# tkoz0/linear-program-solver

Measured on AMD Instinct MI355X. Metric: pivots/sec + achieved HBM GB/s on dense float64 tableau, 1/2/4/8 MI355X, higher is better.
Workload: dtype f64

## Files before the change

include/lpgpu_diag.h:

```cpp
#ifndef LPGPU_DIAG_H
#define LPGPU_DIAG_H

#include "lpgpu.h"

#ifdef __cplusplus
extern "C" {
#endif

int lpdiag_geometry(lp_handle *h, long long *out );

int lpdiag_sweep_buffers(const lp_handle *h, int *nbuf);

int lpdiag_sweep_clocks(lp_handle *h, unsigned long long *out , int cap, int *n);

int lpdiag_sweep_block_clocks(lp_handle *h, unsigned long long *out , int cap, int *n);

int lpdiag_set_xcd_shards(lp_handle *h, int on);

int lpdiag_stamps(lp_handle *h, long long *out );
int lpdiag_bstamps(lp_handle *h, long long *out );

#ifdef __cplusplus
}
#endif

#endif
```

linear-program-solver_amd/csrc/engine.h:

```cpp
#pragma once

#include <hip/hip_runtime.h>
#include <stdint.h>

#include "../../include/lpgpu.h"
#include "geometry.h"

namespace lpk {

constexpr int MODE_RUN = 0;
constexpr int MODE_SOLVE = 1;

constexpr int RATIO_FULL = 0;
constexpr int RATIO_LOCAL = 1;
constexpr int RATIO_CHECK = 2;

constexpr int RSRC_RECORDS = 0;
constexpr int RSRC_GIVEN = 1;
constexpr int RSRC_SLOTS = 2;
constexpr int RSRC_BAND = 3;

constexpr int ST_STRADDLE = 3;

constexpr int PICK_RATIO = 0;
constexpr int PICK_CHECK = 1;
constexpr int PICK_EXPLICIT = 2;
// ... 85 lines not shown
    int gmaj;
    lp_tol tol;
    long long *stamps;
    unsigned long long *gran;
    unsigned spin_max;
    unsigned xwait_ms;
    int fault;
    int hier;
    int rank;
    int xtarget;
    int share;
    int fault_xcc;
    unsigned long long *xbuf;
    unsigned long long *const *peer;
    double *Tout;
    unsigned *dflips;
    unsigned flipseq;
    unsigned long long *sweep_clk;
    unsigned sweep_lseq;
};
constexpr int SWEEP_CLK_RING = 1024;
constexpr int SWEEP_BLK_MAX = 8192;

constexpr int NRANK_MAX = 64;
constexpr long long XS_SUM_PAR = (NRANK_MAX + 1) * 8;
constexpr long long XS_XREP = 2 * XS_SUM_PAR;
constexpr long long XS_PROW = 8 * XS_XREP;
constexpr long long XS_PROW_BLOCK = 2 * 4 * 64;
constexpr long long XS_PROW_RANK = 256 * XS_PROW_BLOCK;
__host__ __device__ inline long long xs_granules(int nranks)
{
    return XS_PROW + 2LL * nranks * XS_PROW_RANK + 256 * 8;
}

hipError_t launch_reset(hipStream_t s, const Args &A, int mode, int rule, int chain, long long cap,
                        long long r, long long c);
hipError_t launch_load_eager(hipStream_t s, const Args &A);
hipError_t launch_enter(hipStream_t s, const Args &A);
hipError_t launch_ratio(hipStream_t s, const Args &A, int t, int grp, int mode, int from_erec,
                        long long check_local_row);
hipError_t launch_pick(hipStream_t s, const Args &A, int t, int mode);
hipError_t launch_gather(hipStream_t s, const Args &A, int t);
hipError_t launch_prow(hipStream_t s, const Args &A, int t, int grp, int rsrc, int peek);
hipError_t launch_sweep(hipStream_t s, const Args &A, int grp, int nd_max, int cnt = -1, hipEvent_t e0 = nullptr,
                        hipEvent_t e1 = nullptr, bool *flipped = nullptr);

constexpr int GRAN_REGIONS = 4;
constexpr long long GRAN_SHARD = (long long)GRAN_REGIONS * GROUP_MAXBLOCKS * 8;
constexpr long long XS_READER_STRIDE = 1032;
constexpr long long GRAN_TOTAL = (XS_SHARDS + 2) * GRAN_SHARD;
GroupGeom group_geom(long long rc, long long ld, long long n, int bmax, int xr, int nshard, int share,
                     bool xs_ok = true);
const void *sel_kernel(int ipl, int nb, bool xr, bool xs);
int persistent_occupancy(const Variant &v);
hipError_t launch_sel(hipStream_t s, const Args &A, const GroupGeom &geo, int grp, int count, int from_erec,
                      unsigned seq, int xr, int first, int fmode, int frule, long long fcap, hipEvent_t e0,
                      hipEvent_t e1);
hipError_t launch_group(hipStream_t s, const Args &A, const GroupGeom &geo, int grp, int count,
                        int from_erec, unsigned seq, int bmax, int xr, const Args *As, int nshard,
                        int first, int fmode, int frule, long long fcap, hipEvent_t e0 = nullptr,
                        hipEvent_t e1 = nullptr);
hipError_t launch_persistent(const void *fn, dim3 grid, void **args, size_t lds, hipStream_t s, hipEvent_t e0,
                             hipEvent_t e1);
hipError_t launch_peer_ping(hipStream_t s, const Args &A, unsigned tag, unsigned flags, int *ok_dev);
hipError_t launch_group_min(hipStream_t s, double *const *ptrs, int n);

struct ColStat {
    double gmin;
// ... 24 lines not shown
```

linear-program-solver_amd/csrc/geometry.h:

```cpp
#pragma once

#include <algorithm>
#include <cstdint>
#include <functional>

#ifdef __HIP__
#define LPK_HD __host__ __device__
#else
#define LPK_HD
#endif

namespace lpk {

constexpr int BMAX = 64;

constexpr int GROUP_MAXBLOCKS = 256;
constexpr int XS_SHARDS = 8;
constexpr int GROUP_MINBLOCKS = 64;
constexpr int GROUP_THREADS = 64;
constexpr int GROUP_MAXRPL = 4;
constexpr long long GROUP_LDS_MAX = 96 * 1024;
LPK_HD inline long long group_lds(long long rc, long long ld, long long g, int count)
{
    const long long rpb = (rc + g - 1) / g, cpb = (ld + g - 1) / g;
// ... 112 lines not shown
            }
        }
        const long long tail = spread ? ((S.rows + nrun * nsg - 1) / (nrun * nsg) + 7) / 8 * 8 : 0;
        return SweepPlan{K, nsg, nrun, run, runb, na, tail, nfull * 64 * WL, ncol, nrun * nsg};
    }
    constexpr int RW = 4;
    const long long ns = (S.ld + 127) / 128;
    const long long slots = (long long)E.cus * bpc;
    const bool tailed = ns >= 2 && (E.tail_mode == 2 || (E.tail_mode == 1 && S.rows * (ns - 1) >= 2048 * slots));
    const long long nsg = tailed ? ns - 1 : ns;
    long long nrun = slots / nsg;
    if (nrun < 1) nrun = 1;
    long long run = (S.rows + nrun - 1) / nrun;
    run = (run + RW - 1) / RW * RW;
    nrun = (S.rows + run - 1) / run;
    const long long tail = tailed ? ((S.rows + nrun * nsg - 1) / (nrun * nsg) + RW - 1) / RW * RW : 0;
    return SweepPlan{K, nsg, nrun, run, run, (int)nrun, tail, 0, 0, nrun * nsg};
}

inline SweepPlan plan_sweep(const SweepShape &S, const SweepEnv &E)
{
    return plan_sweep_grid(S, choose_sweep_kernel(S), E);
}

struct Variant {
    bool sel;
    int nr, ipl;
    int rpl;
    bool xr, xs, hk;
    size_t lds;
};
constexpr int OCC_MISSING = -(1 << 30);
using Occupancy = std::function<int(const Variant &)>;

inline GroupGeom plan_sel(long long rc, long long n, int bmax, int xcd_cus, bool xr, bool xs_ok, int share,
                          const Occupancy &occ)
{
    GroupGeom G;
    if (rc < 1 || n < 1 || bmax < 1 || bmax > BMAX) return G;
    int xs = 0;
    long long rps = rc;
    if ((rc + 63) / 64 > 64) {
        if (!xs_ok || bmax <= 32) return G;
        xs = XS_SHARDS;
        rps = (rc + XS_SHARDS - 1) / XS_SHARDS;
    }
// ... 109 lines not shown
```

linear-program-solver_amd/csrc/kernels.hip:

```cpp
#include "engine.h"
#include "device.h"
#include "knobs.h"

#include <hip/hip_ext.h>

#include <array>
#include <map>
#include <mutex>

namespace lpk {



__global__ void k_reset(Args A, int mode, int rule, int chain, long long cap, long long r,
                        long long c)
{
    Ctl *ctl = A.ctl;
    ctl->status = LP_PIVOTED;
    ctl->mode = mode;
    ctl->rule = rule;
    ctl->chain = chain;
    ctl->cap = cap;
    ctl->r = r;
    ctl->c = c;
// ... 1563 lines not shown
    while (h) {
        int ra32, rb32;
        const int sa = next_pivot_row(h, mysr, ra32);
        const bool two = h != 0;
        const int sb = two ? next_pivot_row(h, mysr, rb32) : sa;
        if (!two) rb32 = ra32;
        const long long ra_ = ra32, rb_ = rb32;
        double ma[NK], mb[NK];
#pragma unroll
        for (int k = 0; k < NK; ++k) {
            ma[k] = M[mq(ra_, 16 * k + (lane & 15))];
            mb[k] = M[mq(rb_, 16 * k + (lane & 15))];
        }
        double ya = P[(long long)sa * ld + col], yb = P[(long long)sb * ld + col];
        fix_chain_dpp<NB>(ya, ma, p, sa);
        if (ok) Tout[ra_ * ld + col] = ya;
        if (two) {
            fix_chain_dpp<NB>(yb, mb, p, sb);
            if (ok) Tout[rb_ * ld + col] = yb;
        }
    }
}

constexpr int SWEEP_LA = 0;
constexpr int SWEEP_LA_T = 0;
constexpr int SWEEP_LA_OOP = 2;
constexpr bool SWEEP_RGQ = true;
template <int W, int NB, int D, int SA>
__global__ void __launch_bounds__(64 * W)
k_sweep_rl(const double *T, double *Tout, const double *__restrict__ P, const double *__restrict__ M,
           const long long *__restrict__ dR, const Ctl *__restrict__ ctl, long long ld, long long rows, int grp,
           int nstrips, long long run, long long tail, long long tcol, long long tend, int nexp,
           unsigned *dflips, unsigned flipseq, unsigned long long *clk, unsigned lseq, long long runb, int na)
{
    constexpr int RW = 8;
    constexpr int NC = NB / 2;
    constexpr int XS = W * RW * 64;
    constexpr int LAT = (SA & 2) ? SWEEP_LA_OOP : SWEEP_LA_T;
    constexpr int SWEEP_QP = 16;
    constexpr int QP = (D * (XS + 2 * 4 * BMAX + SWEEP_QP) * 8 + 8 * NB <= 80 * 1024 || W > 4) ? SWEEP_QP : 0;
    constexpr int MS = 2 * 4 * BMAX + QP;
    static_assert(NB % 2 == 0 && NB <= BMAX && D >= 2 && W >= 4, "k_sweep_rl");
    __shared__ __attribute__((aligned(16))) double xs[D][XS];
    __shared__ __attribute__((aligned(16))) double ms[D][MS];
    __shared__ long long sr[NB];
    constexpr int LDS_BASE = D * (XS + MS) * 8 + NB * 8;
    constexpr int NF = (W <= 4 && LDS_BASE + 64 * (NB * 8 + 4) <= 80 * 1024) ? 64 : 16;
    __shared__ __attribute__((aligned(16))) double fixm[NF][NB];
    __shared__ int fmeta[NF];
    const int nd = (int)ctl->ndef[grp];
    if (nd == 0 || ctl->bar_timeout) return;
    const int lane = threadIdx.x & 63;
    const int wave = __builtin_amdgcn_readfirstlane(threadIdx.x >> 6);
    if (dflips && blockIdx.x == 0 && threadIdx.x == 0) *dflips = flipseq;
    const unsigned long long clk_c0 = __builtin_amdgcn_s_memtime(), clk_r0 = __builtin_amdgcn_s_memrealtime();
    if (threadIdx.x < NB) sr[threadIdx.x] = (int)threadIdx.x < nd ? dR[threadIdx.x] : -2;
    auto srow = [&](int s) -> long long { return sr[s]; };
    const int strip = (int)(blockIdx.x % (unsigned)nstrips);
    const long long ri = (long long)(blockIdx.x / (unsigned)nstrips);
    const long long r0 = ri < na ? ri * run : (long long)na * run + (ri - na) * runb;
    const long long r1 = min(rows, r0 + (ri < na ? run : runb));
    const long long colw = (long long)strip * 64 * W + 64 * wave;
    const long long col = min(colw + (lane & ~1), ld - 2) + (lane & 1);
    const bool cok = colw + lane < ld;
    const long long t0 = (long long)blockIdx.x * tail, t1 = tail > 0 ? min(rows, t0 + tail) : 0;
    const long long tc = min(tcol + lane, ld - 1);
    const bool tok = tcol + lane < ld;
    if (nd != nexp) {
        __syncthreads();
        auto one = [&](long long row, long long c, bool ok) {
            double x = T[row * ld + c];
            for (int s = 0; s < nd; ++s) {
                if (srow(s) == row) x = P[(long long)s * ld + c];
                else x = fma(-M[mq(row, s)], P[(long long)s * ld + c], x);
            }
            if (ok) Tout[row * ld + c] = x;
        };
        for (long long row = r0; row < r1; ++row) one(row, col, cok);
        for (long long row = t0 + wave; row < t1; row += W) one(row, tc, tok);
        return;
    }
    double p[NB];
#pragma unroll
    for (int s = 0; s < NB; ++s) p[s] = P[(long long)s * ld + col];
// ... 120 lines not shown
    for (int f = 0; f < nf; ++f) {
        int meta;
        double mk[NK];
        meta = __builtin_amdgcn_readfirstlane(fmeta[f]);
#pragma unroll
        for (int k = 0; k < NK; ++k) mk[k] = fixm[f][16 * k + (lane & 15)];
        const int s0 = meta & 255;
        double y = pick_p<0, NB, NB>(p, s0);
        fix_chain_dpp<NB>(y, mk, p, s0);
        if (cok) Tout[(r0 + (meta >> 8)) * ld + col] = y;
    }
    if (ovf) fix_rows<NB>(P, M, Tout, ld, col, cok, p, mysr, r0, r1, 0, 0, ovf);
    if (clk && threadIdx.x == 0) {
        const unsigned long long c1 = __builtin_amdgcn_s_memtime(), rt1 = __builtin_amdgcn_s_memrealtime();
        if (blockIdx.x == 0) {
            unsigned long long *e = clk + (lseq % SWEEP_CLK_RING) * 4;
            e[1] = c1 - clk_c0;
            e[2] = rt1 - clk_r0;
            e[3] = clk_r0;
            e[0] = lseq;
        }
        if (blockIdx.x < SWEEP_BLK_MAX) {
            unsigned long long *e = clk + SWEEP_CLK_RING * 4 + blockIdx.x * 4;
            e[0] = lseq;
            e[1] = clk_r0;
            e[2] = rt1;
            e[3] = c1 - clk_c0;
        }
    }
    if (t0 >= t1) return;
    if (tend - tcol <= 4 && t1 - t0 <= 64LL * W) {
        if (64 * wave < t1 - t0) {
            const long long rw = t0 + 64 * wave + lane;
            const bool rok = rw < t1;
            const long long rr = rok ? rw : t1 - 1;
            const int rri = (int)rr;
            double m[NB];
#pragma unroll
            for (int s = 0; s < NB; ++s) m[s] = M[mq(rr, s)];
            const bool tpiv = __ballot(mysr >= t0 && mysr < t1) != 0;
            for (long long c = tcol; c < tend; ++c) {
                double x = T[rr * ld + c];
                const double pv = lane < NB ? P[(long long)lane * ld + c] : 0.0;
                if (tpiv) {
#pragma unroll
                    for (int s = 0; s < NB; ++s) {
                        const double ps = readlane_f64(pv, s);
                        x = rri == __builtin_amdgcn_readlane((int)(unsigned)mysr, s) ? ps : fma(-m[s], ps, x);
                    }
                } else {
// ... 266 lines not shown
    auto it = cache.find(fn);
    if (it != cache.end()) return it->second;
    int n = 0;
    if (hipOccupancyMaxActiveBlocksPerMultiprocessor(&n, fn, threads, 0) != hipSuccess || n < 1) {
        (void)hipGetLastError();
        n = 1;
    }
    cache[fn] = n;
    return n;
}

static const void *sweep_kernel(const SweepKernel &K)
{
    constexpr int SA = 16, WV = 10;
    if (K.rl)
        return K.W == 8 ? (K.oop ? (const void *)&k_sweep_rl<8, 64, 4, SA | 2> : (const void *)&k_sweep_rl<8, 64, 4, SA>)
                        : (K.oop ? (const void *)&k_sweep_rl<4, 64, 2, SA | 2> : (const void *)&k_sweep_rl<4, 64, 2, SA>);
    return K.nb == 16 ? (const void *)&k_sweep_dp2<WV, 16, SA>
         : K.nb == 32 ? (const void *)&k_sweep_dp2<WV, 32, SA>
         : K.nb == 48 ? (const void *)&k_sweep_dp2<WV, 48, SA>
                      : (const void *)&k_sweep_dp2<WV, 64, SA>;
}

hipError_t launch_sweep(hipStream_t s, const Args &A, int grp, int nd_max, int cnt, hipEvent_t e0, hipEvent_t e1,
                        bool *flipped)
{
    if (flipped) *flipped = false;
    const ProcessKnobs &knobs = process_knobs();
    const SweepShape shape{A.rows, A.n, A.ld, nd_max, cnt, A.share, A.Tout && A.Tout != A.T};
    const SweepKernel K = choose_sweep_kernel(shape);
    const void *fn = sweep_kernel(K);
    const SweepEnv env{sweep_grid_cus(), sweep_blocks_per_cu(fn, 64 * K.W), knobs.sweep_tail, knobs.sweep_split};
    SweepPlan pl = plan_sweep_grid(shape, K, env);
    if (K.nexp < K.nb) {
        hipError_t e = hipMemsetAsync(A.P + (long long)K.nexp * A.ld, 0, (size_t)(K.nb - K.nexp) * A.ld * 8, s);
        if (e == hipSuccess)
            e = hipMemset2DAsync(A.MQ + K.nexp * 4, 4 * BMAX * 8, 0, (size_t)(K.nb - K.nexp) * 4 * 8,
                                 (size_t)((A.rows + 3) / 4), s);
        if (e != hipSuccess) return e;
    }
    const dim3 grid((unsigned)pl.grid);
    const double *T = A.T, *Pp = A.P, *Mp = A.MQ;
    double *To = K.oop ? A.Tout : A.T;
    const long long *dRp = A.dR;
    const Ctl *ctlp = A.ctl;
    long long ld = A.ld, rows = A.rows;
    int grpv = grp, nsv = (int)pl.nsg, nexp = K.nexp;
    unsigned *dfl = K.oop ? A.dflips : nullptr;
    unsigned fseq = A.flipseq;
    unsigned long long *clk = A.sweep_clk;
    unsigned lseq = A.sweep_lseq;
    void *args[] = {&T, &To, &Pp, &Mp, &dRp, &ctlp, &ld, &rows, &grpv, &nsv, &pl.run, &pl.tail, &pl.tcol, &pl.tend,
                    &nexp, &dfl, &fseq, &clk, &lseq, &pl.runb, &pl.na};
    const hipError_t err = hipExtLaunchKernel(fn, grid, dim3(64 * K.W), args, 0, s, e0, e1, 0);
    if (err == hipSuccess && flipped) *flipped = K.oop;
    return err != hipSuccess ? err : hipGetLastError();
}

static const void *group_kernel(int nr, int ipl, int rpl, bool xr, bool hk = false)
{
#define X(NRV, IPLV, RPLV)                                                                     \
    if (nr == NRV && ipl == IPLV && rpl == RPLV)                                               \
        return xr ? reinterpret_cast<const void *>(&k_group<NRV, IPLV, RPLV, true>)            \
             : hk ? reinterpret_cast<const void *>(&k_group<NRV, IPLV, RPLV, false, true>)     \
                  : reinterpret_cast<const void *>(&k_group<NRV, IPLV, RPLV, false>);
    GROUP_VARIANTS(X)
#undef X
    return nullptr;
}

static int persistent_per_cu(const void *fn, size_t lds)
{
    int n = 0;
    if (hipOccupancyMaxActiveBlocksPerMultiprocessor(&n, fn, GROUP_THREADS, lds) != hipSuccess) {
        (void)hipGetLastError();
        return 0;
// ... 86 lines not shown
```

linear-program-solver_amd/csrc/knobs.h:

```cpp
#pragma once

#include <cstdio>
#include <cstdlib>
#include <cstring>

#ifndef LPK_TEAM_WAVES
#define LPK_TEAM_WAVES 8
#endif
#ifndef LPK_TEAM_MAX
#define LPK_TEAM_MAX 32
#endif
#ifndef LPK_TEAM_MIN_ELEMS
#define LPK_TEAM_MIN_ELEMS 1024
#endif
#ifndef LPK_TEAM_LP_ELEMS
#define LPK_TEAM_LP_ELEMS 1500
#endif
#ifndef LPK_TEAM_WINDOW
#define LPK_TEAM_WINDOW 64
#endif

namespace lpk {

using KnobLookup = const char *(*)(const char *);

constexpr double SWEEP_SPLIT = 0.62;

struct ProcessKnobs {
    int sweep_oop = 2;
    unsigned long long oop_room_mb = 1024;
    bool oop_fail_alloc = false;
    int sweep_cus = 0;
    int sweep_tail = 1;
    double sweep_split = SWEEP_SPLIT;
    int coop = 0;
    int hier = 1;
    int gmaj = 1;
    bool ld_raw = false;
};

struct HandleKnobs {
    bool persistent = true;
// ... 54 lines not shown
```

linear-program-solver_amd/csrc/lpgpu.cpp:

```cpp
#include <hip/hip_runtime.h>
#include <rccl/rccl.h>

#include <algorithm>
#include <cmath>
#include <cstdio>
#include <cstdlib>
#include <cstring>
#include <memory>
#include <string>
#include <vector>

#include "engine.h"
#include "knobs.h"
#include "../../include/lpgpu_diag.h"

using lpk::Args;
using lpk::Ctl;
using lpk::Rec;

struct Comm;

struct lp_handle {
    int dev = 0;
    hipStream_t s = nullptr;
    bool own_stream = true;
    int64_t m = 0, n = 0, ld = 0;
    int64_t rb = 0, rc = 0;
    int64_t rows = 0;
    double *T = nullptr, *P = nullptr, *M = nullptr, *MQ = nullptr, *row0 = nullptr, *col0 = nullptr;
    double *Tb[2] = {nullptr, nullptr};
    unsigned *dflips = nullptr;
    unsigned flips = 0, hflips = 0;
    unsigned long long *sweep_clk = nullptr;
    unsigned sweep_lseq = 0;
    bool oop = false;
    long long *dR = nullptr, *dC = nullptr;
    lpk::ERec *erec = nullptr;
    int block = 0;
    int block_auto = 0;
    lpk::HandleKnobs knobs;
    int fallbacks = 0;
    long long *stamps = nullptr;
    unsigned long long *gran = nullptr;
    unsigned gseq = 0;
    unsigned long long *xbuf = nullptr;
    unsigned long long **dpeer = nullptr;
    std::vector<void *> ipc_open;
    bool peer_ok = false;
    bool xbuf_fine = false;
    bool xr_xcd = false;
    int xtarget = -1;
    int share = 1;
    int last_path = 0;
    hipStream_t sx = nullptr;
    lpk::ColStat *cstat = nullptr;
    double *cthr = nullptr;
    long long *cfirst = nullptr, *ccount = nullptr, *coffs = nullptr;
// ... 618 lines not shown
    *row_begin = h->rb;
    *row_count = h->rc;
    return LP_PIVOTED;
}

extern "C" int lp_destroy(lp_handle *h)
{
    if (!h) return LP_PIVOTED;
    (void)hipSetDevice(h->dev);
    if (h->s) (void)hipStreamSynchronize(h->s);
    for (hipEvent_t e : h->ev) (void)hipEventDestroy(e);
    if (h->sx) (void)hipStreamSynchronize(h->sx);
    for (void *p : {(void *)h->cstat, (void *)h->cthr, (void *)h->cfirst, (void *)h->ccount,
                    (void *)h->coffs, (void *)h->rowflag})
        if (p) (void)hipFree(p);
    for (void *p : h->ipc_open) (void)hipIpcCloseMemHandle(p);
    if (h->dpeer) (void)hipFree(h->dpeer);
    if (h->xbuf) (void)hipFree(h->xbuf);
    if (h->sx) (void)hipStreamDestroy(h->sx);
    if (h->Tb[0]) (void)hipFree(h->Tb[0]);
    if (h->Tb[1]) (void)hipFree(h->Tb[1]);
    if (h->dflips) (void)hipFree(h->dflips);
    if (h->sweep_clk) (void)hipFree(h->sweep_clk);
    if (h->P) (void)hipFree(h->P);
    if (h->M) (void)hipFree(h->M);
    if (h->MQ) (void)hipFree(h->MQ);
    if (h->row0) (void)hipFree(h->row0);
    if (h->col0) (void)hipFree(h->col0);
    if (h->dR) (void)hipFree(h->dR);
    if (h->dC) (void)hipFree(h->dC);
    if (h->erec) (void)hipFree(h->erec);
    if (h->stamps) (void)hipFree(h->stamps);
    if (h->gran) (void)hipFree(h->gran);
    if (h->ctl) (void)hipFree(h->ctl);
    if (h->hctl) (void)hipHostFree(h->hctl);
    if (h->log) (void)hipFree(h->log);
    if (h->rec) (void)hipFree(h->rec);
    if (h->xg) (void)hipFree(h->xg);
    if (h->xs) (void)hipFree(h->xs);
    if (h->xr) (void)hipFree(h->xr);
    if (h->comm) {
        if (auto g = std::dynamic_pointer_cast<GroupComm>(h->comm)) {
            auto it = std::find(g->all.begin(), g->all.end(), h);
            if (it != g->all.end()) *it = nullptr;
        }
        h->comm.reset();
// ... 110 lines not shown
    if (!h->prof) return LP_PIVOTED;
    if (h->prof_seen[kind]++ % h->prof_every != 0) return LP_PIVOTED;
    if (h->evused + 2 > h->ev.size()) {
        hipEvent_t a, b;
        HCHK(h, hipEventCreate(&a));
        HCHK(h, hipEventCreate(&b));
        h->ev.push_back(a);
        h->ev.push_back(b);
        h->evkind.push_back(0);
    }
    *e0 = h->ev[h->evused];
    *e1 = h->ev[h->evused + 1];
    h->evkind[h->evused / 2] = kind;
    h->evused += 2;
    return LP_PIVOTED;
}

static int launch_sweep_timed(lp_handle *h, const Args &A, int grp, int cnt, bool *flipped)
{
    hipEvent_t e0, e1;
    CALL(prof_slot(h, &e0, &e1, 0));
    Args a = A;
    a.sweep_lseq = h->sweep_lseq;
    HCHK(h, lpk::launch_sweep(h->s, a, grp, block_of(h), cnt, e0, e1, flipped));
    ++h->sweep_lseq;
    return LP_PIVOTED;
}

struct CallStart {
    int first = 0;
    int mode = 0, rule = 0;
    long long cap = -1;
};

static int launch_group_timed(lp_handle *h, const Args &A, const lpk::GroupGeom &geo, int grp, int cnt,
                              int from_erec, int xr, const Args *As, int nshard, const CallStart &cs)
{
    h->gseq = h->gseq % ((1u << 23) - 1) + 1;
    hipEvent_t e0, e1;
    CALL(prof_slot(h, &e0, &e1, 1));
    Args a = A;
    const lpk::HandleKnobs &kn = h->knobs;
    if (kn.fault_launch > 0 && (unsigned)kn.fault_launch == h->gseq) a.fault = kn.fault_t + 1;
    if (kn.fault_xcc > 0 && (unsigned)kn.fault_xcc == h->gseq) a.fault_xcc = 1;
    HCHK(h, lpk::launch_group(h->s, a, geo, grp, cnt, from_erec, h->gseq, block_of(h), xr, As, nshard,
                              cs.first, cs.mode, cs.rule, cs.cap, e0, e1));
    return LP_PIVOTED;
// ... 751 lines not shown
                      hipMemcpyDeviceToHost));
    unsigned long long last = 0;
    bool any = false;
    for (int b = 0; b < lpk::SWEEP_BLK_MAX; ++b) {
        const unsigned long long v = blk[(size_t)b * 4];
        if (v == ~0ull) continue;
        if (!any || v > last) last = v;
        any = true;
    }
    int k = 0;
    for (int b = 0; any && b < lpk::SWEEP_BLK_MAX && k < cap; ++b) {
        const unsigned long long *e = &blk[(size_t)b * 4];
        if (e[0] != last) continue;
        out[4 * k] = (unsigned long long)b;
        out[4 * k + 1] = e[1];
        out[4 * k + 2] = e[2];
        out[4 * k + 3] = e[3];
        ++k;
    }
    *n = k;
    return LP_PIVOTED;
}

extern "C" int lpdiag_sweep_buffers(const lp_handle *h, int *nbuf)
{
    if (!h || !nbuf) return LP_BAD_ARG;
    *nbuf = h->oop ? 2 : 1;
    return LP_PIVOTED;
}

extern "C" int lpdiag_set_xcd_shards(lp_handle *h, int on)
{
    if (!h) return LP_BAD_ARG;
    h->knobs.xs_ok = on != 0;
    h->block_auto = 0;
    return LP_PIVOTED;
}

extern "C" int lpdiag_stamps(lp_handle *h, long long *out)
{
    if (!h || !out || !h->stamps) return LP_BAD_ARG;
    HCHK(h, hipMemcpy(out, h->stamps, lpk::BMAX * 16 * sizeof(long long), hipMemcpyDeviceToHost));
    return LP_PIVOTED;
}
```

linear-program-solver_amd/lpsol_amd/_lib.py:

```python
from __future__ import annotations

import ctypes as C
import os

import numpy as np

HERE = os.path.dirname(os.path.abspath(__file__))
LIB_PATH = os.environ.get("LPGPU_LIB") or os.path.join(HERE, "_lib", "liblpgpu.so")

PIVOTED, OPTIMAL, UNBOUNDED = 0, 1, 2
ZERO_PIVOT, BAD_ARG, DEVICE_ERROR, CAP_REACHED, BAD_PIVOT = -1, -2, -3, -4, -5
OBJ_INCREASED = -6
INFEASIBLE, PHASE1_FAILED = -7, -8
STAGE_PHASE2, STAGE_ARTIFICIAL, STAGE_DRIVE_OUT = 0, 1, 2
STATUS_NAMES = {PIVOTED: "pivoted", OPTIMAL: "optimal", UNBOUNDED: "unbounded",
                ZERO_PIVOT: "zero_pivot", BAD_ARG: "bad_arg", DEVICE_ERROR: "device_error",
                CAP_REACHED: "cap_reached", BAD_PIVOT: "bad_pivot",
                OBJ_INCREASED: "objective_increased", INFEASIBLE: "infeasible",
                PHASE1_FAILED: "phase1_failed"}
PATH_KERNELS, PATH_PERSISTENT, PATH_PEER, PATH_COLLECTIVE = 0, 1, 2, 3
PATH_NAMES = {PATH_KERNELS: "per-pivot kernels", PATH_PERSISTENT: "persistent selection",
              PATH_PEER: "persistent selection, device-side peer exchange",
              PATH_COLLECTIVE: "per-pivot kernels, one collective per pivot"}
RULE_STANDARD, RULE_MIN_INDEX = 0, 1
# ... 334 lines not shown
        d["kernel"] = "none" if d["blocks"] == 0 else "k_sel" if d["sel"] else "k_group"
        d["on_one_xcd"] = bool(d["flags"] & 1)
        d["two_level_engaged"] = bool(d["flags"] & 2)
        d["xcd_shards_engaged"] = bool(d["flags"] & 16)
        return d

    def sweep_buffers(self) -> int:
        nb = C.c_int(0)
        self._check(self.lib.lpdiag_sweep_buffers(self.h, C.byref(nb)), self.h)
        return nb.value

    def sweep_clocks(self, cap: int = 1024) -> np.ndarray:
        buf = (C.c_ulonglong * (4 * cap))()
        n = C.c_int(0)
        self._check(self.lib.lpdiag_sweep_clocks(self.h, buf, C.c_int(cap), C.byref(n)), self.h)
        return np.array(buf[:4 * n.value], dtype=np.uint64).reshape(-1, 4).astype(np.int64)

    def sweep_block_clocks(self, cap: int = 8192) -> np.ndarray:
        buf = (C.c_ulonglong * (4 * cap))()
        n = C.c_int(0)
        self._check(self.lib.lpdiag_sweep_block_clocks(self.h, buf, C.c_int(cap), C.byref(n)), self.h)
        return np.array(buf[:4 * n.value], dtype=np.uint64).reshape(-1, 4).astype(np.int64)

    def set_xcd_shards(self, on: bool):
        self._check(self.lib.lpdiag_set_xcd_shards(self.h, 1 if on else 0), self.h)

    def get_block(self) -> int:
        b = C.c_int()
        self.lib.lp_get_block(self.h, C.byref(b))
        return b.value

    def profile(self, enable: bool, every: int = 1):
        self.lib.lp_profile(self.h, max(1, int(every)) if enable else 0)

    def update_time(self):
        ms, n = C.c_double(), C.c_int64()
        self.lib.lp_update_time(self.h, C.byref(ms), C.byref(n))
        return ms.value, n.value

    PEER_HANDLE_BYTES = 64

    def peer_handle(self) -> bytes:
        buf = C.create_string_buffer(self.PEER_HANDLE_BYTES)
        self._check(self.lib.lp_peer_handle(self.h, buf), self.h)
        return buf.raw

# ... 723 lines not shown
```

Before: 54430.

## Add device-side adaptive row-run rebalancing and XCD-aware block mapping for sweep

Moves the sweep kernel's per-block row ranges into a double-buffered device table. Optionally, the last finishing block rebalances run lengths from each block's measured clock durations, and an XCD-interleaved block-to-slot mapping can also be enabled. Both aim to cut tail imbalance across blocks and XCDs in the tableau update. Both features default off through compile macros. The new code adds a table load per block, stronger stores for the clock records, and a host table setup that can synchronize the stream when the launch geometry changes.

```diff
diff --git a/include/lpgpu_diag.h b/include/lpgpu_diag.h
--- a/include/lpgpu_diag.h
+++ b/include/lpgpu_diag.h
@@ -15,6 +15,11 @@
 
 int lpdiag_sweep_block_clocks(lp_handle *h, unsigned long long *out , int cap, int *n);
 
+int lpdiag_sweep_runs(lp_handle *h, long long *out , int cap, int *n, long long *generation);
+
+int lpdiag_set_sweep_balance(lp_handle *h, int on);
+int lpdiag_set_sweep_map(lp_handle *h, int mode);
+
 int lpdiag_set_xcd_shards(lp_handle *h, int on);
 
 int lpdiag_stamps(lp_handle *h, long long *out );
diff --git a/linear-program-solver_amd/csrc/engine.h b/linear-program-solver_amd/csrc/engine.h
--- a/linear-program-solver_amd/csrc/engine.h
+++ b/linear-program-solver_amd/csrc/engine.h
@@ -2,6 +2,8 @@
 
 #include <hip/hip_runtime.h>
 #include <stdint.h>
+
+#include <vector>
 
 #include "../../include/lpgpu.h"
 #include "geometry.h"
@@ -133,6 +135,18 @@
 constexpr int SWEEP_CLK_RING = 1024;
 constexpr int SWEEP_BLK_MAX = 8192;
 
+struct SweepTable {
+    unsigned *dev = nullptr;
+    size_t cap = 0;
+    unsigned seq = 0;
+    bool filled = false;
+    long long key[10] = {};
+    int balance = -1, xmap = -1;
+    unsigned grid = 0, nsg = 0, nrun = 0;
+    bool xmapped = false, balanced = false;
+    std::vector<long long> stage;
+};
+void sweep_table_free(SweepTable &tab);
 constexpr int NRANK_MAX = 64;
 constexpr long long XS_SUM_PAR = (NRANK_MAX + 1) * 8;
 constexpr long long XS_XREP = 2 * XS_SUM_PAR;
@@ -153,8 +167,8 @@
 hipError_t launch_pick(hipStream_t s, const Args &A, int t, int mode);
 hipError_t launch_gather(hipStream_t s, const Args &A, int t);
 hipError_t launch_prow(hipStream_t s, const Args &A, int t, int grp, int rsrc, int peek);
-hipError_t launch_sweep(hipStream_t s, const Args &A, int grp, int nd_max, int cnt = -1, hipEvent_t e0 = nullptr,
-                        hipEvent_t e1 = nullptr, bool *flipped = nullptr);
+hipError_t launch_sweep(hipStream_t s, const Args &A, SweepTable &tab, int grp, int nd_max, int cnt = -1,
+                        hipEvent_t e0 = nullptr, hipEvent_t e1 = nullptr, bool *flipped = nullptr);
 
 constexpr int GRAN_REGIONS = 4;
 constexpr long long GRAN_SHARD = (long long)GRAN_REGIONS * GROUP_MAXBLOCKS * 8;
diff --git a/linear-program-solver_amd/csrc/geometry.h b/linear-program-solver_amd/csrc/geometry.h
--- a/linear-program-solver_amd/csrc/geometry.h
+++ b/linear-program-solver_amd/csrc/geometry.h
@@ -158,6 +158,159 @@
 {
     return plan_sweep_grid(S, choose_sweep_kernel(S), E);
 }
+
+
+struct SweepSlot {
+    unsigned strip, run;
+};
+LPK_HD inline bool sweep_xmap_ok(long long nrun, int na)
+{
+    return nrun > 0 && nrun % XS_SHARDS == 0 && na % XS_SHARDS == 0;
+}
+LPK_HD inline SweepSlot sweep_block_slot(unsigned b, unsigned nsg, bool xmap)
+{
+    if (!xmap) return SweepSlot{b % nsg, b / nsg};
+    const unsigned x = b % XS_SHARDS, j = b / XS_SHARDS;
+    return SweepSlot{j % nsg, (j / nsg) * XS_SHARDS + x};
+}
+LPK_HD inline unsigned sweep_slot_block(unsigned strip, unsigned run, unsigned nsg, bool xmap)
+{
+    if (!xmap) return run * nsg + strip;
+    return ((run / XS_SHARDS) * nsg + strip) * XS_SHARDS + run % XS_SHARDS;
+}
+
+inline void sweep_static_run(const SweepPlan &pl, long long rows, long long ri, long long *r0, long long *r1)
+{
+    const long long a = ri < pl.na ? ri * pl.run : (long long)pl.na * pl.run + (ri - pl.na) * pl.runb;
+    *r0 = a;
+    *r1 = std::min(rows, a + (ri < pl.na ? pl.run : pl.runb));
+}
+
+constexpr int SWEEP_RW = 8;
+constexpr int SWEEP_BAL_MAX = 1024;
+
+struct SweepBalance {
+    const long long *prev;
+    long long *out;
+    long long rows;
+    unsigned nsg, nrun;
+    bool xmap;
+    unsigned *len, *dn, *sh, *bad;
+    unsigned long long *w, *ss;
+
+    LPK_HD long long batches() const { return (rows + SWEEP_RW - 1) / SWEEP_RW; }
+    LPK_HD long long cap() const { return 2 * ((batches() + nrun - 1) / nrun); }
+    LPK_HD unsigned grid() const { return nsg * nrun; }
+    LPK_HD unsigned blk(unsigned s, unsigned i) const { return sweep_slot_block(s, i, nsg, xmap); }
+
+    LPK_HD void step_a(unsigned b, unsigned long long d) const
+    {
+        const long long r0 = prev[2 * b], r1 = prev[2 * b + 1];
+        const bool ok = r0 >= 0 && r1 > r0 && r1 <= rows && r0 % SWEEP_RW == 0 && d != 0 && d < (1ull << 32);
+        len[b] = ok ? (unsigned)((r1 - r0 + SWEEP_RW - 1) / SWEEP_RW) : 0;
+        dn[b] = ok ? (unsigned)d : 0;
+        if (!ok) *bad = 1;
+    }
+    LPK_HD void step_b(unsigned s) const
+    {
+        unsigned long long dmin = ~0ull;
+        long long at = 0;
+        bool ok = true;
+        for (unsigned i = 0; i < nrun; ++i) {
+            const unsigned b = blk(s, i);
+            ok = ok && prev[2 * b] == at;
+            at += (long long)len[b] * SWEEP_RW;
+            if (dn[b] < dmin) dmin = dn[b];
+        }
+        ok = ok && prev[2 * blk(s, nrun - 1) + 1] == rows && at == batches() * SWEEP_RW;
+        if (!ok || dmin == 0) *bad = 1;
+        ss[s] = dmin;
+    }
+    LPK_HD void step_c(unsigned b) const
+    {
+        const unsigned s = sweep_block_slot(b, nsg, xmap).strip;
+        const unsigned long long q = dn[b] ? (ss[s] << 16) / dn[b] : 0;
+        w[b] = (unsigned long long)len[b] * q;
+    }
+    LPK_HD void step_d(unsigned s) const
+    {
+        unsigned long long W = 0;
+        for (unsigned i = 0; i < nrun; ++i) W += w[blk(s, i)];
+        unsigned k = 0;
+        while ((W >> k) >> 32) ++k;
+        ss[s] = W >> k;
+        sh[s] = k;
+        if ((W >> k) == 0) *bad = 1;
+    }
+    LPK_HD void step_e(unsigned b) const
+    {
+        const unsigned s = sweep_block_slot(b, nsg, xmap).strip;
+        const long long L = len[b];
+        const long long T = ss[s] ? (long long)((unsigned long long)batches() * (w[b] >> sh[s]) / ss[s]) : L;
+        long long N = L + (T - L) / 2;
+        N = N < 1 ? 1 : N > cap() ? cap() : N;
+        dn[b] = (unsigned)N;
+    }
+    LPK_HD void step_f(unsigned s) const
+    {
+        long long sum = 0;
+        for (unsigned i = 0; i < nrun; ++i) sum += dn[blk(s, i)];
+        long long diff = batches() - sum;
+        for (int pass = 0; diff != 0 && pass < 64; ++pass) {
+            const long long mag = diff > 0 ? diff : -diff;
+            const long long step = mag / nrun > 1 ? mag / nrun : 1;
+            for (unsigned i = 0; i < nrun && diff != 0; ++i) {
+                const unsigned b = blk(s, i);
+                const long long N = dn[b];
+                if (diff > 0) {
+                    const long long a = std::min(std::min(step, diff), cap() - N);
+                    if (a > 0) dn[b] = (unsigned)(N + a), diff -= a;
+                } else {
+                    const long long a = std::min(std::min(step, -diff), N - 1);
+                    if (a > 0) dn[b] = (unsigned)(N - a), diff += a;
+                }
+            }
+        }
+        long long at = 0;
+        for (unsigned i = 0; i < nrun; ++i) {
+            const unsigned b = blk(s, i);
+            if (diff != 0) {
+                out[2 * b] = prev[2 * b];
+                out[2 * b + 1] = prev[2 * b + 1];
+                continue;
+            }
+            out[2 * b] = at * SWEEP_RW;
+            at += dn[b];
+            out[2 * b + 1] = std::min(rows, at * SWEEP_RW);
+        }
+    }
+    LPK_HD void keep(unsigned b) const
+    {
+        out[2 * b] = prev[2 * b];
+        out[2 * b + 1] = prev[2 * b + 1];
+    }
+};
+
+#ifndef __HIP_DEVICE_COMPILE__
+inline void balance_sweep_runs(const long long *prev, const unsigned long long *dur, long long rows, unsigned nsg,
+                               unsigned nrun, bool xmap, long long *out)
+{
+    const unsigned grid = nsg * nrun;
+    unsigned bad = 0;
+    unsigned *len = new unsigned[3 * (size_t)grid + nsg];
+    unsigned long long *w = new unsigned long long[(size_t)grid + nsg];
+    const SweepBalance B{prev, out, rows, nsg, nrun, xmap, len, len + grid, len + 2 * (size_t)grid, &bad, w, w + grid};
+    for (unsigned b = 0; b < grid; ++b) B.step_a(b, dur[b]);
+    if (!bad) for (unsigned s = 0; s < nsg; ++s) B.step_b(s);
+    if (!bad) for (unsigned b = 0; b < grid; ++b) B.step_c(b);
+    if (!bad) for (unsigned s = 0; s < nsg; ++s) B.step_d(s);
+    if (!bad) for (unsigned b = 0; b < grid; ++b) B.step_e(b);
+    if (!bad) for (unsigned s = 0; s < nsg; ++s) B.step_f(s);
+    if (bad) for (unsigned b = 0; b < grid; ++b) B.keep(b);
+    delete[] len;
+    delete[] w;
+}
+#endif
 
 struct Variant {
     bool sel;
diff --git a/linear-program-solver_amd/csrc/kernels.hip b/linear-program-solver_amd/csrc/kernels.hip
--- a/linear-program-solver_amd/csrc/kernels.hip
+++ b/linear-program-solver_amd/csrc/kernels.hip
@@ -1609,6 +1609,50 @@
     }
 }
 
+constexpr int SWEEP_BAL_LDS = SWEEP_BAL_MAX * (3 * 4 + 2 * 8) + 16;
+__device__ __noinline__ void sweep_rebalance(unsigned *rt, const unsigned long long *rec, unsigned lseq, int par,
+                                             long long rows, unsigned nsg, bool xmap, unsigned *scratch)
+{
+    const unsigned grid = gridDim.x, nrun = grid / nsg, nt = blockDim.x, t = threadIdx.x;
+    if (grid > (unsigned)SWEEP_BAL_MAX || nrun * nsg != grid) {
+        if (t == 0) st_sc1(rt, 0u);
+        return;
+    }
+    __builtin_amdgcn_fence(__ATOMIC_ACQUIRE, "agent");
+    asm volatile("s_waitcnt vmcnt(0)" ::: "memory");
+    __syncthreads();
+    long long *tab = reinterpret_cast<long long *>(rt + 4);
+    unsigned long long *w = reinterpret_cast<unsigned long long *>(scratch + 4);
+    unsigned *u = reinterpret_cast<unsigned *>(w + 2 * SWEEP_BAL_MAX);
+    const SweepBalance B{tab + (size_t)par * 2 * grid, tab + (size_t)(par ^ 1) * 2 * grid, rows, nsg, nrun, xmap,
+                         u, u + SWEEP_BAL_MAX, u + 2 * SWEEP_BAL_MAX, scratch, w, w + SWEEP_BAL_MAX};
+    if (t == 0) *B.bad = 0;
+    __syncthreads();
+    for (unsigned b = t; b < grid; b += nt) {
+        const unsigned long long *e = rec + (size_t)b * 4;
+        const bool mine = ld_sc1(&e[0]) == (unsigned long long)lseq;
+        const unsigned long long t0 = ld_sc1(&e[1]), t1 = ld_sc1(&e[2]);
+        B.step_a(b, mine ? t1 - t0 : ~0ull);
+    }
+    __syncthreads();
+    if (!*B.bad) for (unsigned s = t; s < nsg; s += nt) B.step_b(s);
+    __syncthreads();
+    if (!*B.bad) for (unsigned b = t; b < grid; b += nt) B.step_c(b);
+    __syncthreads();
+    if (!*B.bad) for (unsigned s = t; s < nsg; s += nt) B.step_d(s);
+    __syncthreads();
+    if (!*B.bad) for (unsigned b = t; b < grid; b += nt) B.step_e(b);
+    __syncthreads();
+    if (!*B.bad) for (unsigned s = t; s < nsg; s += nt) B.step_f(s);
+    else for (unsigned b = t; b < grid; b += nt) B.keep(b);
+    if (t == 0) {
+        const bool moved = !*B.bad;
+        st_sc1(rt, 0u);
+        if (moved) st_sc1(rt + 1, ld_sc1(rt + 1) + 1u);
+    }
+    __syncthreads();
+}
+
 constexpr int SWEEP_LA = 0;
 constexpr int SWEEP_LA_T = 0;
 constexpr int SWEEP_LA_OOP = 2;
@@ -1618,7 +1662,7 @@
 k_sweep_rl(const double *T, double *Tout, const double *__restrict__ P, const double *__restrict__ M,
            const long long *__restrict__ dR, const Ctl *__restrict__ ctl, long long ld, long long rows, int grp,
            int nstrips, long long run, long long tail, long long tcol, long long tend, int nexp,
-           unsigned *dflips, unsigned flipseq, unsigned long long *clk, unsigned lseq, long long runb, int na)
+           unsigned *dflips, unsigned flipseq, unsigned long long *clk, unsigned lseq, unsigned *rt, int rflags)
 {
     constexpr int RW = 8;
     constexpr int NC = NB / 2;
@@ -1635,6 +1679,8 @@
     constexpr int NF = (W <= 4 && LDS_BASE + 64 * (NB * 8 + 4) <= 80 * 1024) ? 64 : 16;
     __shared__ __attribute__((aligned(16))) double fixm[NF][NB];
     __shared__ int fmeta[NF];
+    __shared__ int bal_last;
+    static_assert(NF < 64 || sizeof(fixm) >= SWEEP_BAL_LDS, "sweep_rebalance's scratch");
     const int nd = (int)ctl->ndef[grp];
     if (nd == 0 || ctl->bar_timeout) return;
     const int lane = threadIdx.x & 63;
@@ -1643,10 +1689,10 @@
     const unsigned long long clk_c0 = __builtin_amdgcn_s_memtime(), clk_r0 = __builtin_amdgcn_s_memrealtime();
     if (threadIdx.x < NB) sr[threadIdx.x] = (int)threadIdx.x < nd ? dR[threadIdx.x] : -2;
     auto srow = [&](int s) -> long long { return sr[s]; };
-    const int strip = (int)(blockIdx.x % (unsigned)nstrips);
-    const long long ri = (long long)(blockIdx.x / (unsigned)nstrips);
-    const long long r0 = ri < na ? ri * run : (long long)na * run + (ri - na) * runb;
-    const long long r1 = min(rows, r0 + (ri < na ? run : runb));
+    const int strip = (int)sweep_block_slot(blockIdx.x, (unsigned)nstrips, (rflags & 1) != 0).strip;
+    const long long *rtab = reinterpret_cast<const long long *>(rt + 4) + (size_t)((rflags >> 2) & 1) * 2 * gridDim.x;
+    const long long r0 = rtab[2 * blockIdx.x];
+    const long long r1 = rtab[2 * blockIdx.x + 1];
     const long long colw = (long long)strip * 64 * W + 64 * wave;
     const long long col = min(colw + (lane & ~1), ld - 2) + (lane & 1);
     const bool cok = colw + lane < ld;
@@ -1813,10 +1859,23 @@
         }
         if (blockIdx.x < SWEEP_BLK_MAX) {
             unsigned long long *e = clk + SWEEP_CLK_RING * 4 + blockIdx.x * 4;
-            e[0] = lseq;
-            e[1] = clk_r0;
-            e[2] = rt1;
-            e[3] = c1 - clk_c0;
+            st_sc1(&e[0], (unsigned long long)lseq);
+            st_sc1(&e[1], clk_r0);
+            st_sc1(&e[2], rt1);
+            st_sc1(&e[3], c1 - clk_c0);
+        }
+    }
+    if constexpr (W == 4 && NF == 64) {
+        if (rflags & 2) {
+            if (threadIdx.x == 0) {
+                drain_stores();
+                const unsigned t = __hip_atomic_fetch_add(gp(rt), 1u, __ATOMIC_RELAXED, __HIP_MEMORY_SCOPE_AGENT);
+                bal_last = t == gridDim.x - 1;
+            }
+            __syncthreads();
+            if (bal_last)
+                sweep_rebalance(rt, clk + SWEEP_CLK_RING * 4, lseq, (rflags >> 2) & 1, rows, (unsigned)nstrips,
+                                (rflags & 1) != 0, reinterpret_cast<unsigned *>(&fixm[0][0]));
         }
     }
     if (t0 >= t1) return;
@@ -2129,8 +2188,57 @@
                       : (const void *)&k_sweep_dp2<WV, 64, SA>;
 }
 
-hipError_t launch_sweep(hipStream_t s, const Args &A, int grp, int nd_max, int cnt, hipEvent_t e0, hipEvent_t e1,
-                        bool *flipped)
+void sweep_table_free(SweepTable &tab)
+{
+    if (tab.dev) (void)hipFree(tab.dev);
+    tab.dev = nullptr;
+    tab.cap = 0;
+    tab.filled = false;
+}
+
+static hipError_t sweep_table_prepare(hipStream_t s, const Args &A, SweepTable &tab, const SweepKernel &K,
+                                      const SweepPlan &pl, int *rflags)
+{
+    const bool solo = K.W == 4 && A.share <= 1;
+    const bool xmap = (tab.xmap < 0 ? LPK_SWEEP_XMAP != 0 : tab.xmap != 0) && solo && sweep_xmap_ok(pl.nrun, pl.na);
+    const bool bal = (tab.balance < 0 ? LPK_SWEEP_BALANCE != 0 : tab.balance != 0) && solo &&
+                     A.sweep_clk && pl.grid <= SWEEP_BAL_MAX && pl.grid <= SWEEP_BLK_MAX && pl.nrun >= 2;
+    *rflags = (xmap ? 1 : 0) | (bal ? 2 : 0) | ((tab.seq++ & 1) ? 4 : 0);
+    const long long key[10] = {pl.grid, pl.nsg, pl.nrun, pl.run, pl.runb, pl.na, A.rows, xmap, bal, 1};
+    tab.grid = (unsigned)pl.grid;
+    tab.nsg = (unsigned)pl.nsg;
+    tab.nrun = (unsigned)pl.nrun;
+    tab.xmapped = xmap;
+    tab.balanced = bal;
+    if (tab.filled && std::equal(key, key + 10, tab.key)) return hipSuccess;
+    hipError_t e = tab.filled ? hipStreamSynchronize(s) : hipSuccess;
+    if (e != hipSuccess) return e;
+    const size_t grid = (size_t)pl.grid;
+    if (tab.cap < grid) {
+        sweep_table_free(tab);
+        e = hipMalloc(&tab.dev, 16 + 4 * grid * sizeof(long long));
+        if (e != hipSuccess) return e;
+        tab.cap = grid;
+    }
+    tab.stage.assign(2 + 4 * grid, 0);
+    for (size_t b = 0; b < grid; ++b) {
+        const SweepSlot sl = sweep_block_slot((unsigned)b, (unsigned)pl.nsg, xmap);
+        long long r0, r1;
+        sweep_static_run(pl, A.rows, sl.run, &r0, &r1);
+        for (size_t t = 0; t < 2; ++t) {
+            tab.stage[2 + t * 2 * grid + 2 * b] = r0;
+            tab.stage[2 + t * 2 * grid + 2 * b + 1] = r1;
+        }
+    }
+    e = hipMemcpyAsync(tab.dev, tab.stage.data(), tab.stage.size() * sizeof(long long), hipMemcpyHostToDevice, s);
+    if (e != hipSuccess) return e;
+    std::copy(key, key + 10, tab.key);
+    tab.filled = true;
+    return hipSuccess;
+}
+
+hipError_t launch_sweep(hipStream_t s, const Args &A, SweepTable &tab, int grp, int nd_max, int cnt, hipEvent_t e0,
+                        hipEvent_t e1, bool *flipped)
 {
     if (flipped) *flipped = false;
     const ProcessKnobs &knobs = process_knobs();
@@ -2139,6 +2247,11 @@
     const void *fn = sweep_kernel(K);
     const SweepEnv env{sweep_grid_cus(), sweep_blocks_per_cu(fn, 64 * K.W), knobs.sweep_tail, knobs.sweep_split};
     SweepPlan pl = plan_sweep_grid(shape, K, env);
+    int rflags = 0;
+    if (K.rl) {
+        const hipError_t e = sweep_table_prepare(s, A, tab, K, pl, &rflags);
+        if (e != hipSuccess) return e;
+    }
     if (K.nexp < K.nb) {
         hipError_t e = hipMemsetAsync(A.P + (long long)K.nexp * A.ld, 0, (size_t)(K.nb - K.nexp) * A.ld * 8, s);
         if (e == hipSuccess)
@@ -2157,8 +2270,9 @@
     unsigned fseq = A.flipseq;
     unsigned long long *clk = A.sweep_clk;
     unsigned lseq = A.sweep_lseq;
+    unsigned *rt = tab.dev;
     void *args[] = {&T, &To, &Pp, &Mp, &dRp, &ctlp, &ld, &rows, &grpv, &nsv, &pl.run, &pl.tail, &pl.tcol, &pl.tend,
-                    &nexp, &dfl, &fseq, &clk, &lseq, &pl.runb, &pl.na};
+                    &nexp, &dfl, &fseq, &clk, &lseq, &rt, &rflags};
     const hipError_t err = hipExtLaunchKernel(fn, grid, dim3(64 * K.W), args, 0, s, e0, e1, 0);
     if (err == hipSuccess && flipped) *flipped = K.oop;
     return err != hipSuccess ? err : hipGetLastError();
diff --git a/linear-program-solver_amd/csrc/knobs.h b/linear-program-solver_amd/csrc/knobs.h
--- a/linear-program-solver_amd/csrc/knobs.h
+++ b/linear-program-solver_amd/csrc/knobs.h
@@ -18,6 +18,13 @@
 #endif
 #ifndef LPK_TEAM_WINDOW
 #define LPK_TEAM_WINDOW 64
+#endif
+
+#ifndef LPK_SWEEP_BALANCE
+#define LPK_SWEEP_BALANCE 0
+#endif
+#ifndef LPK_SWEEP_XMAP
+#define LPK_SWEEP_XMAP 0
 #endif
 
 namespace lpk {
diff --git a/linear-program-solver_amd/csrc/lpgpu.cpp b/linear-program-solver_amd/csrc/lpgpu.cpp
--- a/linear-program-solver_amd/csrc/lpgpu.cpp
+++ b/linear-program-solver_amd/csrc/lpgpu.cpp
@@ -33,6 +33,7 @@
     unsigned flips = 0, hflips = 0;
     unsigned long long *sweep_clk = nullptr;
     unsigned sweep_lseq = 0;
+    lpk::SweepTable sweep_tab;
     bool oop = false;
     long long *dR = nullptr, *dC = nullptr;
     lpk::ERec *erec = nullptr;
@@ -697,6 +698,7 @@
     if (h->Tb[1]) (void)hipFree(h->Tb[1]);
     if (h->dflips) (void)hipFree(h->dflips);
     if (h->sweep_clk) (void)hipFree(h->sweep_clk);
+    lpk::sweep_table_free(h->sweep_tab);
     if (h->P) (void)hipFree(h->P);
     if (h->M) (void)hipFree(h->M);
     if (h->MQ) (void)hipFree(h->MQ);
@@ -853,7 +855,7 @@
     CALL(prof_slot(h, &e0, &e1, 0));
     Args a = A;
     a.sweep_lseq = h->sweep_lseq;
-    HCHK(h, lpk::launch_sweep(h->s, a, grp, block_of(h), cnt, e0, e1, flipped));
+    HCHK(h, lpk::launch_sweep(h->s, a, h->sweep_tab, grp, block_of(h), cnt, e0, e1, flipped));
     ++h->sweep_lseq;
     return LP_PIVOTED;
 }
@@ -1651,6 +1653,45 @@
     return LP_PIVOTED;
 }
 
+extern "C" int lpdiag_sweep_runs(lp_handle *h, long long *out, int cap, int *n, long long *generation)
+{
+    if (!h || !out || !n || !generation || cap < 0) return LP_BAD_ARG;
+    *n = 0;
+    *generation = 0;
+    const lpk::SweepTable &tab = h->sweep_tab;
+    if (!tab.filled) return LP_PIVOTED;
+    HCHK(h, hipSetDevice(h->dev));
+    HCHK(h, hipStreamSynchronize(h->s));
+    const size_t grid = tab.grid;
+    std::vector<long long> buf(2 + 4 * grid);
+    HCHK(h, hipMemcpy(buf.data(), tab.dev, buf.size() * sizeof(long long), hipMemcpyDeviceToHost));
+    *generation = (long long)((unsigned long long)buf[0] >> 32);
+    const long long *t = buf.data() + 2 + (size_t)(tab.seq & 1) * 2 * grid;
+    int k = 0;
+    for (size_t b = 0; b < grid && k < cap; ++b, ++k) {
+        const lpk::SweepSlot sl = lpk::sweep_block_slot((unsigned)b, tab.nsg, tab.xmapped);
+        out[4 * k] = sl.strip;
+        out[4 * k + 1] = sl.run;
+        out[4 * k + 2] = t[2 * b];
+        out[4 * k + 3] = t[2 * b + 1];
+    }
+    *n = k;
+    return LP_PIVOTED;
+}
+
+extern "C" int lpdiag_set_sweep_balance(lp_handle *h, int on)
+{
+    if (!h) return LP_BAD_ARG;
+    h->sweep_tab.balance = on < 0 ? -1 : on != 0;
+    return LP_PIVOTED;
+}
+extern "C" int lpdiag_set_sweep_map(lp_handle *h, int mode)
+{
+    if (!h) return LP_BAD_ARG;
+    h->sweep_tab.xmap = mode < 0 ? -1 : mode != 0;
+    return LP_PIVOTED;
+}
+
 extern "C" int lpdiag_sweep_buffers(const lp_handle *h, int *nbuf)
 {
     if (!h || !nbuf) return LP_BAD_ARG;
diff --git a/linear-program-solver_amd/csrc/sweep_balance_check.cpp b/linear-program-solver_amd/csrc/sweep_balance_check.cpp
--- /dev/null
+++ b/linear-program-solver_amd/csrc/sweep_balance_check.cpp
@@ -0,0 +1,140 @@
+#include <cstdio>
+#include <cstdlib>
+#include <iostream>
+#include <map>
+#include <sstream>
+#include <string>
+#include <vector>
+
+#include "geometry.h"
+
+using namespace lpk;
+
+namespace {
+
+std::map<std::string, std::string> g_fields;
+
+const std::string &field(const char *name)
+{
+    auto it = g_fields.find(name);
+    if (it == g_fields.end()) {
+        std::fprintf(stderr, "sweep_balance_check: field %s missing\n", name);
+        std::exit(2);
+    }
+    return it->second;
+}
+long long num(const char *name) { return std::atoll(field(name).c_str()); }
+
+template <typename T>
+std::vector<T> list(const char *name)
+{
+    std::vector<T> out;
+    std::stringstream ss(field(name));
+    std::string tok;
+    while (std::getline(ss, tok, ',')) out.push_back((T)std::strtoull(tok.c_str(), nullptr, 10));
+    return out;
+}
+
+template <typename V>
+void put(const char *name, const V &v)
+{
+    std::printf(" %s=", name);
+    for (size_t i = 0; i < v.size(); ++i) std::printf(i ? ",%lld" : "%lld", (long long)v[i]);
+}
+
+void do_map()
+{
+    const unsigned nsg = (unsigned)num("nsg"), nrun = (unsigned)num("nrun");
+    const bool xmap = num("xmap") != 0 && sweep_xmap_ok(nrun, (int)num("na"));
+    std::vector<long long> strip, run, back;
+    for (unsigned b = 0; b < nsg * nrun; ++b) {
+        const SweepSlot s = sweep_block_slot(b, nsg, xmap);
+        strip.push_back(s.strip);
+        run.push_back(s.run);
+        back.push_back(sweep_slot_block(s.strip, s.run, nsg, xmap));
+    }
+    std::printf("xmap=%d", (int)xmap);
+    put("strip", strip);
+    put("run", run);
+    put("back", back);
+    std::printf("\n");
+}
+
+void do_fill()
+{
+    const SweepShape S{num("rows"), num("n"), num("ld"), 64, -1, 1, false};
+    const SweepEnv E{(int)num("cus"), (int)num("bpc"), 1, std::atof(field("split").c_str())};
+    const SweepKernel K = choose_sweep_kernel(S);
+    const SweepPlan pl = plan_sweep_grid(S, K, E);
+    const bool xmap = K.rl && num("xmap") != 0 && sweep_xmap_ok(pl.nrun, pl.na);
+    std::vector<long long> strip, run, r0, r1;
+    for (long long b = 0; K.rl && b < pl.grid; ++b) {
+        const SweepSlot s = sweep_block_slot((unsigned)b, (unsigned)pl.nsg, xmap);
+        long long a, e;
+        sweep_static_run(pl, S.rows, s.run, &a, &e);
+        strip.push_back(s.strip);
+        run.push_back(s.run);
+        r0.push_back(a);
+        r1.push_back(e);
+    }
+    std::printf("rl=%d nsg=%lld nrun=%lld na=%d xmap=%d", (int)K.rl, pl.nsg, pl.nrun, pl.na, (int)xmap);
+    put("strip", strip);
+    put("run", run);
+    put("r0", r0);
+    put("r1", r1);
+    std::printf("\n");
+}
+
+void do_balance()
+{
+    const unsigned nsg = (unsigned)num("nsg"), nrun = (unsigned)num("nrun");
+    const std::vector<long long> r0 = list<long long>("r0"), r1 = list<long long>("r1");
+    const std::vector<unsigned long long> dur = list<unsigned long long>("dur");
+    const size_t grid = (size_t)nsg * nrun;
+    if (r0.size() != grid || r1.size() != grid || dur.size() != grid) {
+        std::fprintf(stderr, "sweep_balance_check: lists of %zu, %zu, %zu for %zu blocks\n", r0.size(), r1.size(),
+                     dur.size(), grid);
+        std::exit(2);
+    }
+    std::vector<long long> prev(2 * grid), out(2 * grid, -1);
+    for (size_t b = 0; b < grid; ++b) {
+        prev[2 * b] = r0[b];
+        prev[2 * b + 1] = r1[b];
+    }
+    balance_sweep_runs(prev.data(), dur.data(), num("rows"), nsg, nrun, num("xmap") != 0, out.data());
+    std::vector<long long> o0(grid), o1(grid);
+    for (size_t b = 0; b < grid; ++b) {
+        o0[b] = out[2 * b];
+        o1[b] = out[2 * b + 1];
+    }
+    std::printf("ok=1");
+    put("r0", o0);
+    put("r1", o1);
+    std::printf("\n");
+}
+
+}
+
+int main()
+{
+    std::string line;
+    while (std::getline(std::cin, line)) {
+        std::stringstream ss(line);
+        std::string what, kv;
+        ss >> what;
+        g_fields.clear();
+        while (ss >> kv) {
+            const size_t eq = kv.find('=');
+            if (eq == std::string::npos) continue;
+            g_fields[kv.substr(0, eq)] = kv.substr(eq + 1);
+        }
+        if (what == "map") do_map();
+        else if (what == "fill") do_fill();
+        else if (what == "balance") do_balance();
+        else {
+            std::fprintf(stderr, "sweep_balance_check: request %s\n", what.c_str());
+            return 2;
+        }
+    }
+    return 0;
+}
diff --git a/linear-program-solver_amd/lpsol_amd/_lib.py b/linear-program-solver_amd/lpsol_amd/_lib.py
--- a/linear-program-solver_amd/lpsol_amd/_lib.py
+++ b/linear-program-solver_amd/lpsol_amd/_lib.py
@@ -380,6 +380,18 @@
         self._check(self.lib.lpdiag_sweep_block_clocks(self.h, buf, C.c_int(cap), C.byref(n)), self.h)
         return np.array(buf[:4 * n.value], dtype=np.uint64).reshape(-1, 4).astype(np.int64)
 
+    def sweep_runs(self, cap: int = 8192):
+        buf = (C.c_longlong * (4 * cap))()
+        n, gen = C.c_int(0), C.c_longlong(0)
+        self._check(self.lib.lpdiag_sweep_runs(self.h, buf, C.c_int(cap), C.byref(n), C.byref(gen)), self.h)
+        return np.array(buf[:4 * n.value], dtype=np.int64).reshape(-1, 4), gen.value
+
+    def set_sweep_balance(self, on: int):
+        self._check(self.lib.lpdiag_set_sweep_balance(self.h, int(on)), self.h)
+
+    def set_sweep_map(self, mode: int):
+        self._check(self.lib.lpdiag_set_sweep_map(self.h, int(mode)), self.h)
+
     def set_xcd_shards(self, on: bool):
         self._check(self.lib.lpdiag_set_xcd_shards(self.h, 1 if on else 0), self.h)
 
```

New measurement: 54360. About the same (-0.1%).
